# kongqg/marl-sat

Measured on NVIDIA B200. Metric: SATEnv env-steps/s, uf100-430, 1/2/4/8 B200; achieved HBM GB/s vs peak, higher is better.
Workload: dtype u32

## Files before the change

marl_sat_b200/csrc/internal.h:

```cpp
#pragma once
#include <atomic>

#include "common.cuh"

namespace msat {

constexpr int kCtaThreads = 256;
constexpr int kMaxSmemOptin = 227 * 1024;

struct GroupLayout {
    int rec, st, satw, satw_old, x, smx, tt, stage, bar, misc, total;
};
constexpr int kCfStageClauses = 256;
constexpr int kCfStageBytes = 12 * kCfStageClauses + 16;
inline GroupLayout group_layout(const Dims& d, bool obs) {
    GroupLayout L;
    int o = 0;
    const int noobs_rec = d.lits_bytes > d.csr_bytes ? d.lits_bytes : d.csr_bytes;
    L.rec = o;  o += ((obs ? d.rec_copy_bytes : noobs_rec) + 127) & ~127;
    L.st = o;   o += 4 * d.state_words;
    L.stage = o; o += obs ? 0 : kCfStageBytes;
    L.satw = o; o += 4 * d.sw;
    L.satw_old = o; o += 4 * d.sw;
    L.x = o;    o += obs ? 4 * d.xw : 0;
    L.tt = o;   o += ((2 * d.n + 4) & ~3) + 4;
    o = (o + 7) & ~7;
    L.smx = o;  o += obs ? 8 * (d.fw + 2) : 0;
    L.bar = o;  o += 8;
    L.misc = o; o += 16 + 128;
    L.total = (o + 127) & ~127;
    return L;
}

}

struct msat_plan {
    msat::Dims d;
    int group_threads;
    int group_smem_bytes;
    int smem_bytes;
    int group_threads_noobs;
    int smem_bytes_noobs;
    msat::GroupLayout layout_obs, layout_noobs;
    int compile_smem_bytes;
    int requested_group_threads = 0;
    int reward_mode = 0;
    float r_gamma = 0.99f, r_clause = 0.02f, r_sat = 1.0f;
    unsigned long long* reset_counter = nullptr;
    int obs_i8 = 0;
    mutable std::atomic<unsigned long long> prepared_devices{0};
    mutable std::atomic<unsigned long long> prepared_walksat{0};
};

namespace msat {

constexpr int kMaxFusedSteps = 64;

struct EnvArgs {
    GroupLayout L;
    const uint8_t* bank;
    int P;
    const uint32_t* state_in;
    uint32_t* state_out;
    const int32_t* actions;
    const int32_t* prob_idx;
    const uint32_t* keys;
    const uint32_t* rng_in;
    uint32_t* chain_out;
    uint32_t Bg, env_off;
    int auto_reset;
    int32_t* obs;
    int32_t* gnn_assign;
    float* gnn_cf;
    float* reward;
    int reward_cols;
    uint8_t* done;
    int done_cols;
    uint8_t* solved;
    int32_t* num_unsat;
    int32_t* episode_step;
    int B;
    int num_steps;
    long long act_step_stride;
    int emit_every_step;
    int reward_mode;
    float r_gamma, r_clause, r_sat;
    int32_t* newly_sat;
    unsigned long long* reset_count;
    int obs_i8;
    const int32_t* assign_in;
    const int32_t* step_in;
    const uint8_t* done_in;
};

enum EnvMode { MODE_RESET = 0, MODE_STEP = 1, MODE_OBS = 2, MODE_IMPORT = 3 };

extern int g_gae_force_plain;
extern int g_gae_variant;
extern int g_gae_pipe_min_cols;
extern int g_gae_warps_per_sm;

struct ExportArgs {
    const uint8_t* bank;
    int P;
    const uint32_t* state;
    int B;
    int32_t* assign;
    uint8_t* sat;
    int32_t* num_unsat;
    int32_t* step;
    uint8_t* done;
    int32_t* clauses;
// ... 71 lines not shown
```

marl_sat_b200/csrc/satenv.cu:

```cuda
#include <type_traits>

#include "internal.h"

namespace msat {

__global__ void __launch_bounds__(256) compile_bank_kernel(Dims d, const int32_t* __restrict__ clauses,
                                                           uint8_t* __restrict__ bank) {
    extern __shared__ uint32_t csm[];
    uint32_t* clause_agents = csm;
    uint32_t* var_agents = csm + d.m * d.agw;
    const int tid = threadIdx.x, nt = blockDim.x;
    const int32_t* cl = clauses + (size_t)blockIdx.x * d.m * d.k;
    uint8_t* rec = bank + (size_t)blockIdx.x * d.rec_bytes;
    uint16_t* lits = reinterpret_cast<uint16_t*>(rec);
    uint32_t* mflat = reinterpret_cast<uint32_t*>(rec + d.lits_bytes);

    for (int i = tid; i < (d.m + d.n) * d.agw; i += nt) csm[i] = 0u;
    for (int i = tid; i < d.lits_bytes / 2; i += nt) lits[i] = lit_pad(d);
    for (int i = d.lits_bytes / 4 + d.fw + 1 + tid; i < d.rec_bytes / 4; i += nt)
        reinterpret_cast<uint32_t*>(rec)[i] = 0u;
    __syncthreads();

    for (int c = tid; c < d.m; c += nt) {
        uint32_t* ca = clause_agents + c * d.agw;
// ... 22 lines not shown
            const int v = code >> 1;
            for (int w = 0; w < d.agw; ++w) {
                const uint32_t x = clause_agents[c * d.agw + w];
                if (x) atomicOr(&var_agents[v * d.agw + w], x);
            }
        }
    }
    __syncthreads();
    for (int w = tid; w < d.fw + 1; w += nt) {
        uint32_t bits = 0u;
        for (int b = 0; b < 32; ++b) {
            const int j = w * 32 + b;
            if (j >= d.AD) break;
            const int a = j / d.D, p = j - a * d.D;
            uint32_t bit;
            if (p < d.n) {
                bit = var_to_agent(d, p) == a;
            } else if (p < d.n + d.m) {
                bit = (clause_agents[(p - d.n) * d.agw + (a >> 5)] >> (a & 31)) & 1u;
            } else {
                const int v = p - d.n - d.m;
                bit = ((var_agents[v * d.agw + (a >> 5)] >> (a & 31)) & 1u) && var_to_agent(d, v) != a;
            }
            bits |= bit << b;
        }
        mflat[w] = bits;
    }
    if (d.cnt_words) {
        int* cnt = reinterpret_cast<int*>(csm + (d.m + d.n) * d.agw);
        uint16_t* row_off = reinterpret_cast<uint16_t*>(rec + d.csr_off);
        uint16_t* occ = row_off + ((d.n + 1 + 7) & ~7);
        __syncthreads();
        for (int i = tid; i <= d.n; i += nt) cnt[i] = 0;
        __syncthreads();
        for (int i = tid; i < d.m * d.k; i += nt) {
            const uint32_t code = lits[lit_index(d.ms, i / d.k, i % d.k)];
            if (code != lit_pad(d)) atomicAdd(&cnt[code >> 1], 1);
        }
        __syncthreads();
        if (tid == 0) {
            int run = 0;
            for (int v = 0; v < d.n; ++v) {
                const int c = cnt[v];
                cnt[v] = run;
                row_off[v] = (uint16_t)run;
                run += c;
            }
            row_off[d.n] = (uint16_t)run;
        }
        __syncthreads();
        for (int v = tid; v < d.n; v += nt) {
            int o = cnt[v];
            for (int i = 0; i < d.m * d.k; ++i) {
                const int c = i / d.k;
                const uint32_t code = lits[lit_index(d.ms, c, i - c * d.k)];
                if (code != lit_pad(d) && (int)(code >> 1) == v) occ[o++] = (uint16_t)((c << 1) | (code & 1u));
            }
        }
    }
}


template <int GS>
__device__ __forceinline__ void build_truth_table(const Dims& d, const uint32_t* assign, uint8_t* tt, int gt) {
    const int n2 = 2 * d.n;
    for (int w = gt; 4 * w <= n2; w += GS) {
        const int v = 2 * w;
        const uint32_t word = assign[v >> 5] >> (v & 31);
        const uint32_t a0 = word & 1u, a1 = (word >> 1) & 1u;
        uint32_t b = a0 | ((a0 ^ 1u) << 8) | (a1 << 16) | ((a1 ^ 1u) << 24);
        if (v >= d.n) b = 0u;
        else if (v + 1 >= d.n) b &= 0x0000FFFFu;
        reinterpret_cast<uint32_t*>(tt)[w] = b;
    }
}


template <int GS>
__device__ __forceinline__ void publish_unsat(const Dims& d, int* nunsat, int nsat, int gt) {
    if (GS <= 32) *nunsat = d.m - nsat;
    else if ((gt & 31) == 0 && nsat) atomicAdd(nunsat, -nsat);
}

__device__ __forceinline__ void tma_store_1d(void* gmem_dst, const void* smem_src, uint32_t bytes) {
    asm volatile("cp.async.bulk.global.shared::cta.bulk_group [%0], [%1], %2;" ::"l"(gmem_dst), "r"(smem_u32(smem_src)),
                 "r"(bytes)
                 : "memory");
}
__device__ __forceinline__ void tma_store_commit() { asm volatile("cp.async.bulk.commit_group;" ::: "memory"); }
__device__ __forceinline__ void tma_store_wait_read() { asm volatile("cp.async.bulk.wait_group.read 0;" ::: "memory"); }
__device__ __forceinline__ void tma_store_wait() { asm volatile("cp.async.bulk.wait_group 0;" ::: "memory"); }


template <bool K3>
__device__ __forceinline__ uint32_t true_literals(const Dims& d, const uint16_t* lits, const uint8_t* tt, int c) {
    if (K3) {
        const uint32_t l0 = lits[c], l1 = lits[d.ms + c], l2 = lits[2 * d.ms + c];
        return (uint32_t)tt[l0] + tt[l1] + tt[l2];
    }
    uint32_t cnt = 0u;
#pragma unroll 4
    for (int j = 0; j < d.k; ++j) cnt += tt[lits[lit_index(d.ms, c, j)]];
    return cnt;
}

template <bool K3, bool INCR, bool STORE = true>
__device__ __forceinline__ uint32_t clause_count(const Dims& d, const uint16_t* lits, const uint8_t* tt,
                                                 uint32_t* cntw, int c) {
    if (INCR) return (cntw[c >> 3] >> (4 * (c & 7))) & 15u;
    const uint32_t cnt = true_literals<K3>(d, lits, tt, c);
    if (STORE && cntw && cnt) atomicOr(&cntw[c >> 3], cnt << (4 * (c & 7)));
    return cnt;
}

template <int GS, bool K3, bool INCR, bool STORE>
__device__ __forceinline__ void eval_clauses_gnn(const Dims& d, const uint16_t* lits, const uint8_t* tt, uint32_t* cntw,
                                                 uint32_t* satw, int* nunsat, const float2* cf01, uint8_t* stage,
                                                 float* __restrict__ cf_out, int gid, int gt) {
    const int lane = gt & 31;
    int nsat = 0;
    constexpr int kRoundsPerPass = kCfStageClauses / 32;
    const int full = d.m >> 5;
    for (int w0 = 0; w0 < d.sw; w0 += kRoundsPerPass) {
        const int c0 = w0 * 32;
        const int c1 = min(d.m, c0 + kCfStageClauses);
        uint8_t* gdst = reinterpret_cast<uint8_t*>(cf_out + 3 * (size_t)c0);
        const uint32_t phase16 = (uint32_t)(reinterpret_cast<uintptr_t>(gdst) & 15u);
        if (w0 > 0) {
            if (gt == 0) tma_store_wait_read();
            group_sync<GS>(gid);
        }
        const int wend = min(d.sw, w0 + kRoundsPerPass);
        float* o = reinterpret_cast<float*>(stage + phase16) + 3 * (32 * (gt >> 5) + lane);
        int w = w0 + (gt >> 5);
        for (; w < min(wend, full); w += GS / 32, o += 3 * GS) {
            const uint32_t cnt = clause_count<K3, INCR, STORE>(d, lits, tt, cntw, w * 32 + lane);
            const float2 f = cf01[cnt];
            o[0] = f.x;
            o[1] = f.y;
            o[2] = 1.0f;
            const uint32_t word = __ballot_sync(0xffffffffu, cnt != 0u);
            nsat += __popc(word);
            if (lane == 0) satw[w] = word;
        }
        if (w < wend) {
            const int c = w * 32 + lane;
            uint32_t cnt = 0u;
            if (c < d.m) {
                cnt = clause_count<K3, INCR, STORE>(d, lits, tt, cntw, c);
                const float2 f = cf01[cnt];
                o[0] = f.x;
                o[1] = f.y;
                o[2] = 1.0f;
            }
            const uint32_t word = __ballot_sync(0xffffffffu, cnt != 0u);
            nsat += __popc(word);
            if (lane == 0) satw[w] = word;
        }
        fence_proxy_async();
        group_sync<GS>(gid);
        const uint32_t len = 12u * (uint32_t)(c1 - c0);
        uint32_t head = (16u - phase16) & 15u;
        head = head < len ? head : len;
        const uint32_t body = (len - head) & ~15u;
        if (gt == 0 && body) {
            tma_store_1d(gdst + head, stage + phase16 + head, body);
            tma_store_commit();
        }
        if (gt >= 1 && gt < 8) {
            const uint32_t i = gt < 4 ? (uint32_t)(gt - 1) * 4u : head + body + (uint32_t)(gt - 4) * 4u;
            const bool mine = gt < 4 ? i < head : i < len;
            if (mine) *reinterpret_cast<float*>(gdst + i) = *reinterpret_cast<const float*>(stage + phase16 + i);
        }
    }
    publish_unsat<GS>(d, nunsat, nsat, gt);
}

template <int GS, bool CF>
__device__ __forceinline__ void eval_clauses_pairs(const Dims& d, const uint16_t* lits, const uint8_t* tt, int* nunsat,
                                                   const float2* cf01, uint8_t* stage, float* __restrict__ cf_out,
                                                   int gid, int gt) {
    const uint32_t* l32 = reinterpret_cast<const uint32_t*>(lits);
    const int ms2 = d.ms >> 1;
    int nsat = 0;
    auto counts = [&](int pp, uint32_t& ca, uint32_t& cb) {
        const uint32_t w0 = l32[pp], w1 = l32[ms2 + pp], w2 = l32[2 * ms2 + pp];
        ca = (uint32_t)tt[w0 & 0xFFFFu] + tt[w1 & 0xFFFFu] + tt[w2 & 0xFFFFu];
        cb = (uint32_t)tt[w0 >> 16] + tt[w1 >> 16] + tt[w2 >> 16];
        nsat += (ca != 0u) + (cb != 0u);
    };
    if constexpr (!CF) {
        const int npairs = (d.m + 1) >> 1;
        for (int pp = gt; pp < npairs; pp += GS) {
            uint32_t ca, cb;
            counts(pp, ca, cb);
        }
    } else {
        for (int c0 = 0; c0 < d.m; c0 += kCfStageClauses) {
            const int c1 = min(d.m, c0 + kCfStageClauses);
            uint8_t* gdst = reinterpret_cast<uint8_t*>(cf_out + 3 * (size_t)c0);
            const uint32_t phase16 = (uint32_t)(reinterpret_cast<uintptr_t>(gdst) & 15u);
            if (c0 > 0) {
                if (gt == 0) tma_store_wait_read();
                group_sync<GS>(gid);
            }
            const int npass = (c1 - c0 + 1) >> 1;
            const int p0 = c0 >> 1;
            if ((phase16 & 7u) == 0u) {
                for (int q = gt; q < npass; q += GS) {
                    uint32_t ca, cb;
                    counts(p0 + q, ca, cb);
                    const float2 f = cf01[ca], g = cf01[cb];
                    float2* o = reinterpret_cast<float2*>(stage + phase16 + 24 * q);
                    o[0] = f;
                    o[1] = make_float2(1.0f, g.x);
                    o[2] = make_float2(g.y, 1.0f);
                }
            } else {
                for (int q = gt; q < npass; q += GS) {
                    uint32_t ca, cb;
                    counts(p0 + q, ca, cb);
                    const float2 f = cf01[ca], g = cf01[cb];
                    float* o = reinterpret_cast<float*>(stage + phase16 + 24 * q);
                    o[0] = f.x; o[1] = f.y; o[2] = 1.0f;
                    o[3] = g.x; o[4] = g.y; o[5] = 1.0f;
                }
            }
            fence_proxy_async();
            group_sync<GS>(gid);
            const uint32_t len = 12u * (uint32_t)(c1 - c0);
            uint32_t head = (16u - phase16) & 15u;
            head = head < len ? head : len;
            const uint32_t body = (len - head) & ~15u;
            if (gt == 0 && body) {
                tma_store_1d(gdst + head, stage + phase16 + head, body);
                tma_store_commit();
            }
            if (gt >= 1 && gt < 8) {
                const uint32_t i = gt < 4 ? (uint32_t)(gt - 1) * 4u : head + body + (uint32_t)(gt - 4) * 4u;
                const bool mine = gt < 4 ? i < head : i < len;
                if (mine) *reinterpret_cast<float*>(gdst + i) = *reinterpret_cast<const float*>(stage + phase16 + i);
            }
        }
    }
    nsat = __reduce_add_sync(0xffffffffu, nsat);
    if (nunsat) publish_unsat<GS>(d, nunsat, nsat, gt);
}

template <int GS, bool K3, bool INCR, bool STORE>
__device__ __forceinline__ void eval_clauses_impl(const Dims& d, const uint16_t* lits, const uint8_t* tt, uint32_t* cntw,
                                                  uint32_t* satw, int* nunsat, int gt) {
    const int lane = gt & 31;
    int nsat = 0;
    if constexpr (GS < 32) {
        using piece_t = typename std::conditional<GS == 16, uint16_t, uint8_t>::type;
        piece_t* piece = reinterpret_cast<piece_t*>(satw);
        const uint32_t sh = subwarp_shift<GS>();
        const uint32_t mask = subwarp_mask<GS>();
        const int full = d.m / GS;
        int r = 0;
        for (; r < full; ++r) {
            const uint32_t cnt = clause_count<K3, INCR, STORE>(d, lits, tt, cntw, r * GS + gt);
            const uint32_t bits = (__ballot_sync(mask, cnt != 0u) >> sh) & ((1u << GS) - 1u);
            nsat += __popc(bits);
            if (gt == 0) piece[r] = (piece_t)bits;
        }
        if (full * GS < d.m) {
            const int c = r * GS + gt;
            const uint32_t cnt = c < d.m ? clause_count<K3, INCR, STORE>(d, lits, tt, cntw, c) : 0u;
            const uint32_t bits = (__ballot_sync(mask, cnt != 0u) >> sh) & ((1u << GS) - 1u);
            nsat += __popc(bits);
            if (gt == 0) piece[r] = (piece_t)bits;
            ++r;
        }
        if (gt == 0)
            for (; r < (32 / GS) * d.sw; ++r) piece[r] = 0;
    } else {
        for (int w = gt >> 5; w < d.sw; w += GS / 32) {
            const int c = w * 32 + lane;
            const uint32_t cnt = c < d.m ? clause_count<K3, INCR, STORE>(d, lits, tt, cntw, c) : 0u;
            const uint32_t word = __ballot_sync(0xffffffffu, cnt != 0u);
            nsat += __popc(word);
            if (lane == 0) satw[w] = word;
        }
    }
    if (nunsat) publish_unsat<GS>(d, nunsat, nsat, gt);
}
__device__ __forceinline__ uint32_t spread16(uint32_t x) {
    x = (x | (x << 8)) & 0x00FF00FFu;
    x = (x | (x << 4)) & 0x0F0F0F0Fu;
    x = (x | (x << 2)) & 0x33333333u;
    return (x | (x << 1)) & 0x55555555u;
}
__device__ __forceinline__ void eval_clauses_pairs16(const Dims& d, const uint16_t* lits, const uint8_t* tt,
                                                     uint32_t* satw, int* nunsat, int gt) {
    const uint32_t* l32 = reinterpret_cast<const uint32_t*>(lits);
    const int ms2 = d.ms >> 1;
    const uint32_t sh = subwarp_shift<16>();
    const uint32_t mask = subwarp_mask<16>();
    int nsat = 0;
    for (int w = 0; w < d.sw; ++w) {
        const int pp = 16 * w + gt;
        uint32_t ca = 0u, cb = 0u;
        if (pp < ms2) {
            const uint32_t w0 = l32[pp], w1 = l32[ms2 + pp], w2 = l32[2 * ms2 + pp];
            ca = (uint32_t)tt[w0 & 0xFFFFu] + tt[w1 & 0xFFFFu] + tt[w2 & 0xFFFFu];
            cb = (uint32_t)tt[w0 >> 16] + tt[w1 >> 16] + tt[w2 >> 16];
        }
        const uint32_t ev = (__ballot_sync(mask, ca != 0u) >> sh) & 0xFFFFu;
        const uint32_t od = (__ballot_sync(mask, cb != 0u) >> sh) & 0xFFFFu;
        const uint32_t word = spread16(ev) | (spread16(od) << 1);
        nsat += __popc(word);
        if (gt == 0) satw[w] = word;
    }
    if (nunsat) publish_unsat<16>(d, nunsat, nsat, gt);
}

template <int GS, bool K3, bool INCR>
__device__ __forceinline__ void eval_clauses(const Dims& d, const uint16_t* lits, const uint8_t* tt, uint32_t* cntw,
                                             uint32_t* satw, int* nunsat, int gt) {
    if constexpr (GS == 16 && K3 && !INCR) {
        if (!cntw && d.sw >= 4) {
            eval_clauses_pairs16(d, lits, tt, satw, nunsat, gt);
            return;
// ... 144 lines not shown
        smx[w] = make_uint2(mw, xw);
    }
    group_sync<GS>(gid);

    if constexpr (I8) {
        int8_t* out8 = reinterpret_cast<int8_t*>(obs) + (g_start - s);
        const int lo = s, hi = s + d.AD;
        const int q_lo = (lo + 15) >> 4, q_hi = hi >> 4;
        {
            int q = q_lo + gt;
            const int sh = (q & 1) * 16;
            const uint2* sp = smx + (q >> 1);
            uint4* op = reinterpret_cast<uint4*>(out8) + q;
#pragma unroll 2
            for (; q < q_hi; q += GS, sp += GS / 2, op += GS) {
                const uint2 mx = *sp;
                const uint32_t m16 = mx.x >> sh, x16 = mx.y >> sh;
                __stcs(op, make_uint4(expand_nibble_i8(m16 & 0xFu, x16 & 0xFu),
                                      expand_nibble_i8((m16 >> 4) & 0xFu, (x16 >> 4) & 0xFu),
                                      expand_nibble_i8((m16 >> 8) & 0xFu, (x16 >> 8) & 0xFu),
                                      expand_nibble_i8((m16 >> 12) & 0xFu, (x16 >> 12) & 0xFu)));
            }
        }
        const int head_end = min(16 * q_lo, hi);
        const int tail_start = max(16 * q_hi, head_end);
        auto put = [&](int i) {
            const uint2 mx = smx[i >> 5];
            out8[i] = ((mx.x >> (i & 31)) & 1u) ? (int8_t)((mx.y >> (i & 31)) & 1u) : (int8_t)-1;
        };
        for (int i = lo + gt; i < head_end; i += GS) put(i);
        for (int i = tail_start + gt; i < hi; i += GS) put(i);
        return;
    }
    int32_t* out = obs + (g_start - s);
    const int lo_valid = s, hi_valid = s + d.AD;
    const int q_lo = (lo_valid + 3) >> 2;
    const int q_hi = hi_valid >> 2;
    {
        int q = q_lo + gt;
        const int sh = (q & 7) * 4;
        const uint2* sp = smx + (q >> 3);
        int4* op = reinterpret_cast<int4*>(out) + q;
#pragma unroll 4
        for (; q < q_hi; q += GS, sp += GS / 8, op += GS) {
            const uint2 mx = *sp;
            __stcs(op, expand_nibble((mx.x >> sh) & 0xFu, (mx.y >> sh) & 0xFu));
        }
    }
    if (gt < 8) {
        const int q = (gt < 4) ? q_lo - 1 : q_hi;
        const int i = 4 * q + (gt & 3);
        const bool partial = (gt < 4) ? (4 * q_lo != lo_valid) : (4 * q_hi != hi_valid);
        if (partial && q >= 0 && i >= lo_valid && i < hi_valid) {
            const uint2 mx = smx[i >> 5];
            out[i] = ((mx.x >> (i & 31)) & 1u) ? (int)((mx.y >> (i & 31)) & 1u) : -1;
        }
    }
}

template <int GS, typename F>
__device__ __forceinline__ void store_words_vec4(uint32_t* __restrict__ dst, int count, int gt, F f) {
    int head = (int)(((16u - (uint32_t)(reinterpret_cast<uintptr_t>(dst) & 15u)) & 15u) >> 2);
    head = head < count ? head : count;
    const int n4 = (count - head) >> 2;
    uint4* d4 = reinterpret_cast<uint4*>(dst + head);
    for (int q = gt; q < n4; q += GS) {
        const int i = head + 4 * q;
        __stcs(d4 + q, make_uint4(f(i), f(i + 1), f(i + 2), f(i + 3)));
    }
    if (gt < head) dst[gt] = f(gt);
    const int i = head + 4 * n4 + gt;
    if (gt < 3 && i < count) dst[i] = f(i);
}

template <int GS>
__device__ __forceinline__ void emit_gnn_assignment(const Dims& d, long long row, const uint32_t* assign,
                                                    int32_t* __restrict__ gnn_assign, int gt) {
    store_words_vec4<GS>(reinterpret_cast<uint32_t*>(gnn_assign) + row * d.n, d.n, gt,
                         [&](int v) { return (assign[v >> 5] >> (v & 31)) & 1u; });
}

template <int GS, bool INCR, bool OBS>
__device__ __forceinline__ void run_eval(const Dims& d, const uint16_t* lits, const uint8_t* tt, uint32_t* cntw,
                                         uint32_t* satw, int* nunsat, const float2* cf01, uint8_t* stage, float* cf_row,
                                         bool pairs, int gid, int gt) {
    if constexpr (!OBS && !INCR && GS >= 32) {
        if (pairs) {
            if (cf_row) eval_clauses_pairs<GS, true>(d, lits, tt, nunsat, cf01, stage, cf_row, gid, gt);
            else eval_clauses_pairs<GS, false>(d, lits, tt, nunsat, cf01, stage, cf_row, gid, gt);
            return;
        }
    }
    if (GS >= 32 && cf_row) {
        if constexpr (GS >= 32) {
            const bool store = !INCR && cntw != nullptr;
            if (d.k == 3) {
                if (store) eval_clauses_gnn<GS, true, INCR, true>(d, lits, tt, cntw, satw, nunsat, cf01, stage, cf_row, gid, gt);
                else eval_clauses_gnn<GS, true, INCR, false>(d, lits, tt, cntw, satw, nunsat, cf01, stage, cf_row, gid, gt);
            } else {
                if (store) eval_clauses_gnn<GS, false, INCR, true>(d, lits, tt, cntw, satw, nunsat, cf01, stage, cf_row, gid, gt);
                else eval_clauses_gnn<GS, false, INCR, false>(d, lits, tt, cntw, satw, nunsat, cf01, stage, cf_row, gid, gt);
            }
        }
    } else {
        if (d.k == 3) eval_clauses<GS, true, INCR>(d, lits, tt, cntw, satw, nunsat, gt);
        else eval_clauses<GS, false, INCR>(d, lits, tt, cntw, satw, nunsat, gt);
    }
}

__device__ __forceinline__ void rng_advance(uint32_t& r0, uint32_t& r1) {
    uint32_t a[2], b[2];
    split2(r0, r1, a, b);
    split2(a[0], a[1], a, b);
    uint32_t x0 = 0u, x1 = 3u, y0 = 1u, y1 = 4u;
    threefry2x32(a[0], a[1], x0, x1);
    threefry2x32(a[0], a[1], y0, y1);
    r0 = x0;
    r1 = y0;
}

template <int GS, int MODE, bool OBS, bool MULTI, bool INCR>
__global__ void __launch_bounds__(kCtaThreads, (MULTI || !OBS) ? 4 : 8) env_kernel(const Dims d, const EnvArgs a) {
    extern __shared__ __align__(128) uint8_t smem_raw[];
    constexpr int NG = kCtaThreads / GS;
    constexpr bool FRESH = MODE == MODE_RESET || MODE == MODE_IMPORT;
    const int gid = threadIdx.x / GS, gt = threadIdx.x % GS;
    const int e = blockIdx.x * NG + gid;
    const GroupLayout& L = a.L;
    const int K = MULTI ? a.num_steps : 1;

    uint32_t* s_chain = reinterpret_cast<uint32_t*>(smem_raw + (size_t)NG * L.total);
    if (MULTI && a.rng_in) {
        if (threadIdx.x == 0) {
            uint32_t r0 = a.rng_in[0], r1 = a.rng_in[1];
            for (int j = 0; j < K; ++j) {
                s_chain[10 * j] = r0;
                s_chain[10 * j + 1] = r1;
                rng_advance(r0, r1);
            }
        }
        __syncthreads();
        if ((int)threadIdx.x < K) {
            uint32_t c[10];
            rng_chain_compute(s_chain[10 * threadIdx.x], s_chain[10 * threadIdx.x + 1], c);
            for (int i = 0; i < 10; ++i) s_chain[10 * threadIdx.x + i] = c[i];
        }
        __syncthreads();
        if (blockIdx.x == 0 && threadIdx.x < 10) a.chain_out[threadIdx.x] = s_chain[10 * (K - 1) + threadIdx.x];
    }
    if (e >= a.B) return;

    uint8_t* base = smem_raw + (size_t)gid * L.total;
    uint8_t* rec = base + L.rec;
    uint32_t* st = reinterpret_cast<uint32_t*>(base + L.st);
    uint32_t* satw = reinterpret_cast<uint32_t*>(base + L.satw);
    uint32_t* satw_old = reinterpret_cast<uint32_t*>(base + L.satw_old);
    uint32_t* X = reinterpret_cast<uint32_t*>(base + L.x);
    uint2* smx = reinterpret_cast<uint2*>(base + L.smx);
    uint8_t* tt = base + L.tt;
    uint8_t* stage = base + L.stage;
    uint64_t* bar = reinterpret_cast<uint64_t*>(base + L.bar);
    int* misc = reinterpret_cast<int*>(base + L.misc);
    const uint16_t* lits = reinterpret_cast<const uint16_t*>(rec);
    const uint32_t* mflat = reinterpret_cast<const uint32_t*>(rec + d.lits_bytes);
    uint32_t* st_tail = st + d.aw;
    const uint32_t tma_bytes = OBS ? (uint32_t)d.rec_copy_bytes : (uint32_t)d.lits_bytes;
    uint32_t* cntw = d.cnt_words ? st + d.aw + 4 : nullptr;
    uint32_t* cnt_store = (MODE != MODE_OBS) ? cntw : nullptr;
    const bool want_cf = !OBS && a.gnn_cf != nullptr;
    const bool pairs = !OBS && d.k == 3 && cnt_store == nullptr && cntw == nullptr && a.reward_mode == 0;
    float2* cf01 = reinterpret_cast<float2*>(misc + 4);

    const uint4* sin = FRESH ? nullptr : reinterpret_cast<const uint4*>(a.state_in + (size_t)e * d.state_words);
    const int sw4 = d.state_words >> 2;
    uint4 s0 = make_uint4(0u, 0u, 0u, 0u);
    if (!FRESH && gt < sw4) s0 = sin[gt];
    if constexpr (GS < 32) {
        if (gt < sw4) reinterpret_cast<uint4*>(st)[gt] = s0;
    }
    int act_pre = 0;
    const bool act_pre_ok = GS >= 32 && MODE == MODE_STEP && !INCR && d.action_mode == 0 && gt < d.A;
    if (act_pre_ok) act_pre = a.actions[(size_t)e * d.A + gt];
    if (gt == 0) {
        misc[0] = d.m;
        mbar_init(bar, 1);
    }
    if (want_cf && gt < 16) cf01[gt] = make_float2(gt > 0 ? 1.0f : 0.0f, __fdiv_rn((float)gt, 3.0f));
    if constexpr (GS >= 32) {
        if (gt < sw4) reinterpret_cast<uint4*>(st)[gt] = s0;
    }
    if (!FRESH) {
#pragma unroll 1
        for (int i = gt + GS; i < sw4; i += GS) reinterpret_cast<uint4*>(st)[i] = sin[i];
    } else {
#pragma unroll 1
        for (int i = gt + GS; i < sw4; i += GS) reinterpret_cast<uint4*>(st)[i] = make_uint4(0u, 0u, 0u, 0u);
    }
    group_sync<GS>(gid);

    int step_cur = (MODE == MODE_RESET) ? 0
                 : (MODE == MODE_IMPORT) ? (a.step_in ? a.step_in[e] : 0) : (int)st_tail[ST_STEP];
    int nunsat_prev = FRESH ? 0 : (int)st_tail[ST_NUNSAT];
    uint32_t flags = (MODE == MODE_RESET) ? 0u
                   : (MODE == MODE_IMPORT) ? ((a.done_in && a.done_in[e]) ? 1u : 0u) : st_tail[ST_FLAGS];
    int pidx;
    if (FRESH) pidx = a.prob_idx[e];
    else pidx = (int)st_tail[ST_PIDX];
    pidx = clamp_problem(pidx, a.P);
    int loaded_pidx = -1;
    bool loaded_csr = false;
    uint32_t phase = 0u;
    int nunsat = nunsat_prev;

    for (int j = 0; j < K; ++j) {
        const bool last = j == K - 1;
        const bool emit = last || a.emit_every_step;
        const long long row = (a.emit_every_step ? (long long)j * a.B : 0LL) + e;
        const long long orow = (long long)j * a.B + e;

        if (!INCR && loaded_pidx != pidx && gt == 0) {
            if (j > 0) fence_proxy_async();
            mbar_expect_tx(bar, tma_bytes);
            tma_load_1d(rec, a.bank + (size_t)pidx * d.rec_bytes, tma_bytes, bar);
        }
        const bool need_csr = INCR && !(loaded_csr && loaded_pidx == pidx);
        if (need_csr && gt == 0) {
            if (j > 0) fence_proxy_async();
            mbar_expect_tx(bar, (uint32_t)d.csr_bytes);
            tma_load_1d(rec, a.bank + (size_t)pidx * d.rec_bytes + d.csr_off, (uint32_t)d.csr_bytes, bar);
        }
        if (MODE == MODE_STEP && a.reward_mode) {
            if (INCR) {
                run_eval<GS, true, OBS>(d, lits, tt, cntw, satw_old, nullptr, cf01, stage, nullptr, false, gid, gt);
            } else {
                if (loaded_pidx != pidx) {
                    mbar_wait(bar, phase);
                    phase ^= 1u;
                    loaded_pidx = pidx;
                }
                build_truth_table<GS>(d, st, tt, gt);
                group_sync<GS>(gid);
                run_eval<GS, false, OBS>(d, lits, tt, nullptr, satw_old, nullptr, cf01, stage, nullptr, false, gid, gt);
            }
            group_sync<GS>(gid);
        }

        if (MODE == MODE_RESET) {
            threefry_assign<GS>(d, a.keys[2 * (size_t)e], a.keys[2 * (size_t)e + 1], st, gt);
        } else if (MODE == MODE_IMPORT) {
            load_assign<GS>(d, a.assign_in + (size_t)e * d.n, st, gt);
        } else if (MODE == MODE_STEP) {
            if (INCR) {
                if (need_csr) {
                    mbar_wait(bar, phase);
                    phase ^= 1u;
                    loaded_pidx = pidx;
                    loaded_csr = true;
                }
                for_each_flip<GS>(d, a.actions + (long long)j * a.act_step_stride, e, gt, false, 0,
                                  [&](int v) { flip_and_update_counts(d, rec, v, st, cntw); });
            } else {
                for_each_flip<GS>(d, a.actions + (long long)j * a.act_step_stride, e, gt, act_pre_ok && j == 0, act_pre,
                                  [&](int v) { atomicXor(&st[v >> 5], 1u << (v & 31)); });
            }
        }
        if (!INCR && cnt_store)
            for (int i = gt; i < d.cnt_words; i += GS) cnt_store[i] = 0u;
        group_sync<GS>(gid);
        if (!INCR) {
            build_truth_table<GS>(d, st, tt, gt);
            if (loaded_pidx != pidx) {
                mbar_wait(bar, phase);
                phase ^= 1u;
                loaded_pidx = pidx;
            }
            group_sync<GS>(gid);
        }

        float* cf_row = (want_cf && emit) ? a.gnn_cf + row * d.m * 3 : nullptr;
        run_eval<GS, INCR, OBS>(d, lits, tt, INCR ? cntw : cnt_store, satw, &misc[0], cf01, stage, cf_row, pairs, gid, gt);
        group_sync<GS>(gid);
        nunsat = misc[0];

        if (MODE == MODE_STEP) {
            if (!MULTI && a.rng_in && blockIdx.x == 0 && threadIdx.x == 0) {
                uint32_t c[10];
                rng_chain_compute(a.rng_in[0], a.rng_in[1], c);
                for (int i = 0; i < 10; ++i) a.chain_out[i] = c[i];
            }
            const bool solved = nunsat == 0;
            const bool done = solved || (step_cur + 1 >= d.max_steps);
            int newly = 0;
            float r = solved ? 1.0f : 0.0f;
            if (a.reward_mode) {
                for (int w = 0; w < d.sw; ++w) newly += __popc(satw[w] & ~satw_old[w]);
                const float r_pbrs = __fsub_rn(__fmul_rn(a.r_gamma, (float)(-nunsat)), (float)(-nunsat_prev));
                const float r_cl = __fmul_rn((float)newly, a.r_clause);
                r = __fadd_rn(__fadd_rn(r_pbrs, r_cl), solved ? a.r_sat : 0.0f);
            }
            if (a.reward) {
                float* rp = a.reward + orow * a.reward_cols;
#pragma unroll 1
                for (int i = gt; i < a.reward_cols; i += GS) rp[i] = r;
            }
            if (a.done) {
                uint8_t* dp = a.done + orow * a.done_cols;
#pragma unroll 1
                for (int i = gt; i < a.done_cols; i += GS) dp[i] = done ? 1 : 0;
            }
            if (gt == 0) {
                if (a.solved) a.solved[orow] = solved ? 1 : 0;
                if (a.num_unsat) a.num_unsat[orow] = nunsat;
                if (a.episode_step) a.episode_step[orow] = step_cur + 1;
                if (a.newly_sat) a.newly_sat[orow] = newly;
            }
            if (done && a.auto_reset) {
                group_sync<GS>(gid);
                uint32_t rk0, rk1;
                if (a.rng_in) {
                    if (gt < 4) {
                        const int base_lane = GS < 32 ? (int)(threadIdx.x & 31u & (32u - GS)) : 0;
                        uint32_t c6 = 0u, c7 = 0u, c8 = 0u, c9 = 0u, r0 = 0u, r1 = 0u, np, k0, k1;
                        if (MULTI) {
                            c6 = s_chain[10 * j + 6]; c7 = s_chain[10 * j + 7];
                            c8 = s_chain[10 * j + 8]; c9 = s_chain[10 * j + 9];
                        } else {
                            r0 = a.rng_in[0]; r1 = a.rng_in[1];
                        }
                        env_reset_inputs_4lanes(0xFu << base_lane, gt, base_lane, MULTI, r0, r1, c6, c7, c8, c9, a.Bg,
                                                a.env_off + (uint32_t)e, (uint32_t)a.P, np, k0, k1);
                        if (gt == 0) {
                            misc[1] = (int)np;
                            misc[2] = (int)k0;
                            misc[3] = (int)k1;
                        }
                    }
                    group_sync<GS>(gid);
                    pidx = misc[1];
                    rk0 = (uint32_t)misc[2];
                    rk1 = (uint32_t)misc[3];
                } else {
                    pidx = a.prob_idx[e];
                    rk0 = a.keys[2 * (size_t)e];
                    rk1 = a.keys[2 * (size_t)e + 1];
                }
                pidx = clamp_problem(pidx, a.P);
                const bool need_lits = pidx != loaded_pidx || (INCR && loaded_csr);
                if (gt == 0) {
                    misc[0] = d.m;
                    if (a.reset_count) atomicAdd(a.reset_count, 1ULL);
                    if (need_lits) {
                        fence_proxy_async();
                        mbar_expect_tx(bar, tma_bytes);
                        tma_load_1d(rec, a.bank + (size_t)pidx * d.rec_bytes, tma_bytes, bar);
                    }
                }
                for (int i = gt; i < d.aw; i += GS) st[i] = 0u;
                if (cnt_store)
                    for (int i = gt; i < d.cnt_words; i += GS) cnt_store[i] = 0u;
                group_sync<GS>(gid);
                threefry_assign<GS>(d, rk0, rk1, st, gt);
                group_sync<GS>(gid);
                build_truth_table<GS>(d, st, tt, gt);
                if (need_lits) {
                    mbar_wait(bar, phase);
                    phase ^= 1u;
                    loaded_pidx = pidx;
                    loaded_csr = false;
                }
                group_sync<GS>(gid);
                if (cf_row) {
                    if (gt == 0) tma_store_wait();
                    group_sync<GS>(gid);
                }
                run_eval<GS, false, OBS>(d, lits, tt, cnt_store, satw, &misc[0], cf01, stage, cf_row, pairs, gid, gt);
                group_sync<GS>(gid);
                nunsat = misc[0];
                step_cur = 0;
                flags = 0u;
            } else {
                step_cur += 1;
                flags = done ? 1u : 0u;
            }
            nunsat_prev = nunsat;
        }
        if (emit) {
            if (!OBS && a.gnn_assign) emit_gnn_assignment<GS>(d, row, st, a.gnn_assign, gt);
            if (OBS && a.obs) {
                if (a.obs_i8) emit_obs<GS, true>(d, row, st, satw, X, smx, mflat, a.obs, gid, gt);
                else emit_obs<GS, false>(d, row, st, satw, X, smx, mflat, a.obs, gid, gt);
            }
        }
        if (!last) {
            if (cf_row && gt == 0) tma_store_wait_read();
            group_sync<GS>(gid);
            if (gt == 0) misc[0] = d.m;
        }
    }

    if (want_cf && gt == 0) tma_store_wait_read();
    if (MODE != MODE_OBS) {
        group_sync<GS>(gid);
        if (gt == 0) {
            st_tail[ST_STEP] = (uint32_t)step_cur;
            st_tail[ST_PIDX] = (uint32_t)pidx;
            st_tail[ST_NUNSAT] = (uint32_t)nunsat;
            st_tail[ST_FLAGS] = flags;
        }
        group_sync<GS>(gid);
        uint4* sout = reinterpret_cast<uint4*>(a.state_out + (size_t)e * d.state_words);
#pragma unroll 1
        for (int i = gt; i < (d.state_words >> 2); i += GS) sout[i] = reinterpret_cast<const uint4*>(st)[i];
    }
}

template <int GS, bool OBS>
static cudaError_t launch_env_gs(const msat_plan* plan, EnvMode mode, const EnvArgs& a, cudaStream_t s, int smem_bytes) {
    const int groups = kCtaThreads / GS;
    const int grid = (a.B + groups - 1) / groups;
    if (grid == 0) return cudaSuccess;
    constexpr int kFns = OBS ? 5 : 7;
    const void* fns[7] = {(const void*)env_kernel<GS, MODE_RESET, OBS, false, false>,
                          (const void*)env_kernel<GS, MODE_STEP, OBS, false, false>,
                          (const void*)env_kernel<GS, MODE_OBS, OBS, false, false>,
                          (const void*)env_kernel<GS, MODE_IMPORT, OBS, false, false>,
                          (const void*)env_kernel<GS, MODE_STEP, OBS, true, false>,
                          OBS ? nullptr : (const void*)env_kernel<GS, MODE_STEP, false, false, true>,
                          OBS ? nullptr : (const void*)env_kernel<GS, MODE_STEP, false, true, true>};
    const bool multi = mode == MODE_STEP && a.num_steps > 1;
    const bool incr = !OBS && mode == MODE_STEP && plan->d.cnt_words > 0;
    if (multi) smem_bytes += 40 * a.num_steps;
    if (smem_bytes > 48 * 1024) {
        int dev = 0;
        cudaError_t err = cudaGetDevice(&dev);
        if (err != cudaSuccess) return err;
        const unsigned long long bit = 1ULL << ((OBS ? 0 : 32) + (dev & 31));
        if (!(plan->prepared_devices.load(std::memory_order_acquire) & bit)) {
            for (int i = 0; i < kFns; ++i) {
                err = cudaFuncSetAttribute(fns[i], cudaFuncAttributeMaxDynamicSharedMemorySize, kMaxSmemOptin);
                if (err != cudaSuccess) return err;
            }
            plan->prepared_devices.fetch_or(bit, std::memory_order_release);
        }
    }
    const void* fn = fns[incr ? 5 + (int)multi : (multi ? 4 : (int)mode)];
    Dims d = plan->d;
    EnvArgs args = a;
    void* params[] = {&d, &args};
    return cudaLaunchKernel(fn, dim3(grid), dim3(kCtaThreads), params, (size_t)smem_bytes, s);
}

cudaError_t launch_env(const msat_plan* plan, EnvMode mode, const EnvArgs& a0, cudaStream_t s) {
    EnvArgs a = a0;
    if (a.num_steps < 1) a.num_steps = 1;
    const bool noobs = a.obs == nullptr;
    a.L = noobs ? plan->layout_noobs : plan->layout_obs;
    a.obs_i8 = plan->obs_i8;
    const int gs = noobs ? plan->group_threads_noobs : plan->group_threads;
    const int smem = noobs ? plan->smem_bytes_noobs : plan->smem_bytes;
    if (noobs) {
        switch (gs) {
            case 32: return launch_env_gs<32, false>(plan, mode, a, s, smem);
            case 64: return launch_env_gs<64, false>(plan, mode, a, s, smem);
            case 128: return launch_env_gs<128, false>(plan, mode, a, s, smem);
            default: return launch_env_gs<256, false>(plan, mode, a, s, smem);
        }
    }
    switch (gs) {
        case 16: return launch_env_gs<16, true>(plan, mode, a, s, smem);
        case 32: return launch_env_gs<32, true>(plan, mode, a, s, smem);
        case 64: return launch_env_gs<64, true>(plan, mode, a, s, smem);
        case 128: return launch_env_gs<128, true>(plan, mode, a, s, smem);
        default: return launch_env_gs<256, true>(plan, mode, a, s, smem);
    }
}

cudaError_t launch_compile_bank(const msat_plan* plan, const int32_t* clauses, int P, uint8_t* bank, cudaStream_t s) {
    if (P == 0) return cudaSuccess;
    if (plan->compile_smem_bytes > 48 * 1024) {
        cudaError_t err = cudaFuncSetAttribute((const void*)compile_bank_kernel,
                                               cudaFuncAttributeMaxDynamicSharedMemorySize, plan->compile_smem_bytes);
        if (err != cudaSuccess) return err;
    }
// ... 62 lines not shown
```

Baseline: 121.7 million.

## Replace TMA-staged clause-feature stores with direct streaming stores and shrink smem

Clause features for the GNN outputs used to be staged in a shared-memory buffer and written out with bulk-async (TMA) stores, with group syncs and wait-group fences between chunks. They are now written straight to global memory with streaming (__stcs) stores, using float2 stores when the output is 8-byte aligned. This drops the staging buffer and its synchronisation, which shrinks the per-group shared-memory footprint, and the non-obs launch bound is raised from 4 to 6 blocks per SM. Other changes: the cf lookup table now comes from a constant array, and the RNG chain computation moves to kernel entry on the non-obs step path. The cost is scattered 4/8-byte stores in place of coalesced bulk copies, and possible register pressure from the higher occupancy target.

```diff
diff --git a/marl_sat_b200/csrc/internal.h b/marl_sat_b200/csrc/internal.h
--- a/marl_sat_b200/csrc/internal.h
+++ b/marl_sat_b200/csrc/internal.h
@@ -9,17 +9,15 @@
 constexpr int kMaxSmemOptin = 227 * 1024;
 
 struct GroupLayout {
-    int rec, st, satw, satw_old, x, smx, tt, stage, bar, misc, total;
+    int rec, st, satw, satw_old, x, smx, tt, cf, bar, misc, total;
 };
-constexpr int kCfStageClauses = 256;
-constexpr int kCfStageBytes = 12 * kCfStageClauses + 16;
 inline GroupLayout group_layout(const Dims& d, bool obs) {
     GroupLayout L;
     int o = 0;
     const int noobs_rec = d.lits_bytes > d.csr_bytes ? d.lits_bytes : d.csr_bytes;
     L.rec = o;  o += ((obs ? d.rec_copy_bytes : noobs_rec) + 127) & ~127;
     L.st = o;   o += 4 * d.state_words;
-    L.stage = o; o += obs ? 0 : kCfStageBytes;
+    L.cf = o;   o += obs ? 0 : 128;
     L.satw = o; o += 4 * d.sw;
     L.satw_old = o; o += 4 * d.sw;
     L.x = o;    o += obs ? 4 * d.xw : 0;
@@ -27,7 +25,7 @@
     o = (o + 7) & ~7;
     L.smx = o;  o += obs ? 8 * (d.fw + 2) : 0;
     L.bar = o;  o += 8;
-    L.misc = o; o += 16 + 128;
+    L.misc = o; o += 16;
     L.total = (o + 127) & ~127;
     return L;
 }
diff --git a/marl_sat_b200/csrc/satenv.cu b/marl_sat_b200/csrc/satenv.cu
--- a/marl_sat_b200/csrc/satenv.cu
+++ b/marl_sat_b200/csrc/satenv.cu
@@ -128,16 +128,6 @@
     else if ((gt & 31) == 0 && nsat) atomicAdd(nunsat, -nsat);
 }
 
-__device__ __forceinline__ void tma_store_1d(void* gmem_dst, const void* smem_src, uint32_t bytes) {
-    asm volatile("cp.async.bulk.global.shared::cta.bulk_group [%0], [%1], %2;" ::"l"(gmem_dst), "r"(smem_u32(smem_src)),
-                 "r"(bytes)
-                 : "memory");
-}
-__device__ __forceinline__ void tma_store_commit() { asm volatile("cp.async.bulk.commit_group;" ::: "memory"); }
-__device__ __forceinline__ void tma_store_wait_read() { asm volatile("cp.async.bulk.wait_group.read 0;" ::: "memory"); }
-__device__ __forceinline__ void tma_store_wait() { asm volatile("cp.async.bulk.wait_group 0;" ::: "memory"); }
-
-
 template <bool K3>
 __device__ __forceinline__ uint32_t true_literals(const Dims& d, const uint16_t* lits, const uint8_t* tt, int c) {
     if (K3) {
@@ -149,6 +139,11 @@
     for (int j = 0; j < d.k; ++j) cnt += tt[lits[lit_index(d.ms, c, j)]];
     return cnt;
 }
+
+__constant__ float2 kCf01[16] = {{0.f, 0.f / 3.f},  {1.f, 1.f / 3.f},  {1.f, 2.f / 3.f},  {1.f, 3.f / 3.f},
+                                 {1.f, 4.f / 3.f},  {1.f, 5.f / 3.f},  {1.f, 6.f / 3.f},  {1.f, 7.f / 3.f},
+                                 {1.f, 8.f / 3.f},  {1.f, 9.f / 3.f},  {1.f, 10.f / 3.f}, {1.f, 11.f / 3.f},
+                                 {1.f, 12.f / 3.f}, {1.f, 13.f / 3.f}, {1.f, 14.f / 3.f}, {1.f, 15.f / 3.f}};
 
 template <bool K3, bool INCR, bool STORE = true>
 __device__ __forceinline__ uint32_t clause_count(const Dims& d, const uint16_t* lits, const uint8_t* tt,
@@ -161,131 +156,61 @@
 
 template <int GS, bool K3, bool INCR, bool STORE>
 __device__ __forceinline__ void eval_clauses_gnn(const Dims& d, const uint16_t* lits, const uint8_t* tt, uint32_t* cntw,
-                                                 uint32_t* satw, int* nunsat, const float2* cf01, uint8_t* stage,
-                                                 float* __restrict__ cf_out, int gid, int gt) {
+                                                 uint32_t* satw, int* nunsat, const float2* cf01,
+                                                 float* __restrict__ cf_out, int gt) {
     const int lane = gt & 31;
     int nsat = 0;
-    constexpr int kRoundsPerPass = kCfStageClauses / 32;
-    const int full = d.m >> 5;
-    for (int w0 = 0; w0 < d.sw; w0 += kRoundsPerPass) {
-        const int c0 = w0 * 32;
-        const int c1 = min(d.m, c0 + kCfStageClauses);
-        uint8_t* gdst = reinterpret_cast<uint8_t*>(cf_out + 3 * (size_t)c0);
-        const uint32_t phase16 = (uint32_t)(reinterpret_cast<uintptr_t>(gdst) & 15u);
-        if (w0 > 0) {
-            if (gt == 0) tma_store_wait_read();
-            group_sync<GS>(gid);
-        }
-        const int wend = min(d.sw, w0 + kRoundsPerPass);
-        float* o = reinterpret_cast<float*>(stage + phase16) + 3 * (32 * (gt >> 5) + lane);
-        int w = w0 + (gt >> 5);
-        for (; w < min(wend, full); w += GS / 32, o += 3 * GS) {
-            const uint32_t cnt = clause_count<K3, INCR, STORE>(d, lits, tt, cntw, w * 32 + lane);
+    for (int w = gt >> 5; w < d.sw; w += GS / 32) {
+        const int c = w * 32 + lane;
+        uint32_t cnt = 0u;
+        if (c < d.m) {
+            cnt = clause_count<K3, INCR, STORE>(d, lits, tt, cntw, c);
             const float2 f = cf01[cnt];
-            o[0] = f.x;
-            o[1] = f.y;
-            o[2] = 1.0f;
-            const uint32_t word = __ballot_sync(0xffffffffu, cnt != 0u);
-            nsat += __popc(word);
-            if (lane == 0) satw[w] = word;
-        }
-        if (w < wend) {
-            const int c = w * 32 + lane;
-            uint32_t cnt = 0u;
-            if (c < d.m) {
-                cnt = clause_count<K3, INCR, STORE>(d, lits, tt, cntw, c);
-                const float2 f = cf01[cnt];
-                o[0] = f.x;
-                o[1] = f.y;
-                o[2] = 1.0f;
-            }
-            const uint32_t word = __ballot_sync(0xffffffffu, cnt != 0u);
-            nsat += __popc(word);
-            if (lane == 0) satw[w] = word;
-        }
-        fence_proxy_async();
-        group_sync<GS>(gid);
-        const uint32_t len = 12u * (uint32_t)(c1 - c0);
-        uint32_t head = (16u - phase16) & 15u;
-        head = head < len ? head : len;
-        const uint32_t body = (len - head) & ~15u;
-        if (gt == 0 && body) {
-            tma_store_1d(gdst + head, stage + phase16 + head, body);
-            tma_store_commit();
-        }
-        if (gt >= 1 && gt < 8) {
-            const uint32_t i = gt < 4 ? (uint32_t)(gt - 1) * 4u : head + body + (uint32_t)(gt - 4) * 4u;
-            const bool mine = gt < 4 ? i < head : i < len;
-            if (mine) *reinterpret_cast<float*>(gdst + i) = *reinterpret_cast<const float*>(stage + phase16 + i);
-        }
+            __stcs(cf_out + 3 * c, f.x);
+            __stcs(cf_out + 3 * c + 1, f.y);
+            __stcs(cf_out + 3 * c + 2, 1.0f);
+        }
+        const uint32_t word = __ballot_sync(0xffffffffu, cnt != 0u);
+        nsat += __popc(word);
+        if (lane == 0) satw[w] = word;
     }
     publish_unsat<GS>(d, nunsat, nsat, gt);
 }
 
 template <int GS, bool CF>
 __device__ __forceinline__ void eval_clauses_pairs(const Dims& d, const uint16_t* lits, const uint8_t* tt, int* nunsat,
-                                                   const float2* cf01, uint8_t* stage, float* __restrict__ cf_out,
-                                                   int gid, int gt) {
+                                                   const float2* cf01, float* __restrict__ cf_out, int gt) {
     const uint32_t* l32 = reinterpret_cast<const uint32_t*>(lits);
     const int ms2 = d.ms >> 1;
+    const int npairs = (d.m + 1) >> 1;
+    const bool al8 = (reinterpret_cast<uintptr_t>(cf_out) & 7u) == 0u;
     int nsat = 0;
-    auto counts = [&](int pp, uint32_t& ca, uint32_t& cb) {
+    for (int pp = gt; pp < npairs; pp += GS) {
         const uint32_t w0 = l32[pp], w1 = l32[ms2 + pp], w2 = l32[2 * ms2 + pp];
-        ca = (uint32_t)tt[w0 & 0xFFFFu] + tt[w1 & 0xFFFFu] + tt[w2 & 0xFFFFu];
-        cb = (uint32_t)tt[w0 >> 16] + tt[w1 >> 16] + tt[w2 >> 16];
+        const uint32_t ca = (uint32_t)tt[w0 & 0xFFFFu] + tt[w1 & 0xFFFFu] + tt[w2 & 0xFFFFu];
+        const uint32_t cb = (uint32_t)tt[w0 >> 16] + tt[w1 >> 16] + tt[w2 >> 16];
         nsat += (ca != 0u) + (cb != 0u);
-    };
-    if constexpr (!CF) {
-        const int npairs = (d.m + 1) >> 1;
-        for (int pp = gt; pp < npairs; pp += GS) {
-            uint32_t ca, cb;
-            counts(pp, ca, cb);
-        }
-    } else {
-        for (int c0 = 0; c0 < d.m; c0 += kCfStageClauses) {
-            const int c1 = min(d.m, c0 + kCfStageClauses);
-            uint8_t* gdst = reinterpret_cast<uint8_t*>(cf_out + 3 * (size_t)c0);
-            const uint32_t phase16 = (uint32_t)(reinterpret_cast<uintptr_t>(gdst) & 15u);
-            if (c0 > 0) {
-                if (gt == 0) tma_store_wait_read();
-                group_sync<GS>(gid);
-            }
-            const int npass = (c1 - c0 + 1) >> 1;
-            const int p0 = c0 >> 1;
-            if ((phase16 & 7u) == 0u) {
-                for (int q = gt; q < npass; q += GS) {
-                    uint32_t ca, cb;
-                    counts(p0 + q, ca, cb);
-                    const float2 f = cf01[ca], g = cf01[cb];
-                    float2* o = reinterpret_cast<float2*>(stage + phase16 + 24 * q);
-                    o[0] = f;
-                    o[1] = make_float2(1.0f, g.x);
-                    o[2] = make_float2(g.y, 1.0f);
+        if constexpr (CF) {
+            const float2 f = cf01[ca], g = cf01[cb];
+            float* o = cf_out + 6 * pp;
+            const bool two = 2 * pp + 1 < d.m;
+            if (al8) {
+                __stcs(reinterpret_cast<float2*>(o), f);
+                if (two) {
+                    __stcs(reinterpret_cast<float2*>(o) + 1, make_float2(1.0f, g.x));
+                    __stcs(reinterpret_cast<float2*>(o) + 2, make_float2(g.y, 1.0f));
+                } else {
+                    __stcs(o + 2, 1.0f);
                 }
             } else {
-                for (int q = gt; q < npass; q += GS) {
-                    uint32_t ca, cb;
-                    counts(p0 + q, ca, cb);
-                    const float2 f = cf01[ca], g = cf01[cb];
-                    float* o = reinterpret_cast<float*>(stage + phase16 + 24 * q);
-                    o[0] = f.x; o[1] = f.y; o[2] = 1.0f;
-                    o[3] = g.x; o[4] = g.y; o[5] = 1.0f;
+                __stcs(o, f.x);
+                __stcs(o + 1, f.y);
+                __stcs(o + 2, 1.0f);
+                if (two) {
+                    __stcs(o + 3, g.x);
+                    __stcs(o + 4, g.y);
+                    __stcs(o + 5, 1.0f);
                 }
-            }
-            fence_proxy_async();
-            group_sync<GS>(gid);
-            const uint32_t len = 12u * (uint32_t)(c1 - c0);
-            uint32_t head = (16u - phase16) & 15u;
-            head = head < len ? head : len;
-            const uint32_t body = (len - head) & ~15u;
-            if (gt == 0 && body) {
-                tma_store_1d(gdst + head, stage + phase16 + head, body);
-                tma_store_commit();
-            }
-            if (gt >= 1 && gt < 8) {
-                const uint32_t i = gt < 4 ? (uint32_t)(gt - 1) * 4u : head + body + (uint32_t)(gt - 4) * 4u;
-                const bool mine = gt < 4 ? i < head : i < len;
-                if (mine) *reinterpret_cast<float*>(gdst + i) = *reinterpret_cast<const float*>(stage + phase16 + i);
             }
         }
     }
@@ -596,12 +521,12 @@
 
 template <int GS, bool INCR, bool OBS>
 __device__ __forceinline__ void run_eval(const Dims& d, const uint16_t* lits, const uint8_t* tt, uint32_t* cntw,
-                                         uint32_t* satw, int* nunsat, const float2* cf01, uint8_t* stage, float* cf_row,
-                                         bool pairs, int gid, int gt) {
+                                         uint32_t* satw, int* nunsat, const float2* cf01, float* cf_row, bool pairs,
+                                         int gt) {
     if constexpr (!OBS && !INCR && GS >= 32) {
         if (pairs) {
-            if (cf_row) eval_clauses_pairs<GS, true>(d, lits, tt, nunsat, cf01, stage, cf_row, gid, gt);
-            else eval_clauses_pairs<GS, false>(d, lits, tt, nunsat, cf01, stage, cf_row, gid, gt);
+            if (cf_row) eval_clauses_pairs<GS, true>(d, lits, tt, nunsat, cf01, cf_row, gt);
+            else eval_clauses_pairs<GS, false>(d, lits, tt, nunsat, cf01, cf_row, gt);
             return;
         }
     }
@@ -609,11 +534,11 @@
         if constexpr (GS >= 32) {
             const bool store = !INCR && cntw != nullptr;
             if (d.k == 3) {
-                if (store) eval_clauses_gnn<GS, true, INCR, true>(d, lits, tt, cntw, satw, nunsat, cf01, stage, cf_row, gid, gt);
-                else eval_clauses_gnn<GS, true, INCR, false>(d, lits, tt, cntw, satw, nunsat, cf01, stage, cf_row, gid, gt);
+                if (store) eval_clauses_gnn<GS, true, INCR, true>(d, lits, tt, cntw, satw, nunsat, cf01, cf_row, gt);
+                else eval_clauses_gnn<GS, true, INCR, false>(d, lits, tt, cntw, satw, nunsat, cf01, cf_row, gt);
             } else {
-                if (store) eval_clauses_gnn<GS, false, INCR, true>(d, lits, tt, cntw, satw, nunsat, cf01, stage, cf_row, gid, gt);
-                else eval_clauses_gnn<GS, false, INCR, false>(d, lits, tt, cntw, satw, nunsat, cf01, stage, cf_row, gid, gt);
+                if (store) eval_clauses_gnn<GS, false, INCR, true>(d, lits, tt, cntw, satw, nunsat, cf01, cf_row, gt);
+                else eval_clauses_gnn<GS, false, INCR, false>(d, lits, tt, cntw, satw, nunsat, cf01, cf_row, gt);
             }
         }
     } else {
@@ -634,7 +559,7 @@
 }
 
 template <int GS, int MODE, bool OBS, bool MULTI, bool INCR>
-__global__ void __launch_bounds__(kCtaThreads, (MULTI || !OBS) ? 4 : 8) env_kernel(const Dims d, const EnvArgs a) {
+__global__ void __launch_bounds__(kCtaThreads, MULTI ? 4 : (OBS ? 8 : 6)) env_kernel(const Dims d, const EnvArgs a) {
     extern __shared__ __align__(128) uint8_t smem_raw[];
     constexpr int NG = kCtaThreads / GS;
     constexpr bool FRESH = MODE == MODE_RESET || MODE == MODE_IMPORT;
@@ -642,6 +567,12 @@
     const int e = blockIdx.x * NG + gid;
     const GroupLayout& L = a.L;
     const int K = MULTI ? a.num_steps : 1;
+
+    if (!OBS && MODE == MODE_STEP && !MULTI && a.rng_in && blockIdx.x == 0 && threadIdx.x == 0) {
+        uint32_t c[10];
+        rng_chain_compute(a.rng_in[0], a.rng_in[1], c);
+        for (int i = 0; i < 10; ++i) a.chain_out[i] = c[i];
+    }
 
     uint32_t* s_chain = reinterpret_cast<uint32_t*>(smem_raw + (size_t)NG * L.total);
     if (MULTI && a.rng_in) {
@@ -672,7 +603,6 @@
     uint32_t* X = reinterpret_cast<uint32_t*>(base + L.x);
     uint2* smx = reinterpret_cast<uint2*>(base + L.smx);
     uint8_t* tt = base + L.tt;
-    uint8_t* stage = base + L.stage;
     uint64_t* bar = reinterpret_cast<uint64_t*>(base + L.bar);
     int* misc = reinterpret_cast<int*>(base + L.misc);
     const uint16_t* lits = reinterpret_cast<const uint16_t*>(rec);
@@ -683,7 +613,7 @@
     uint32_t* cnt_store = (MODE != MODE_OBS) ? cntw : nullptr;
     const bool want_cf = !OBS && a.gnn_cf != nullptr;
     const bool pairs = !OBS && d.k == 3 && cnt_store == nullptr && cntw == nullptr && a.reward_mode == 0;
-    float2* cf01 = reinterpret_cast<float2*>(misc + 4);
+    float2* cf01 = reinterpret_cast<float2*>(base + L.cf);
 
     const uint4* sin = FRESH ? nullptr : reinterpret_cast<const uint4*>(a.state_in + (size_t)e * d.state_words);
     const int sw4 = d.state_words >> 2;
@@ -699,7 +629,7 @@
         misc[0] = d.m;
         mbar_init(bar, 1);
     }
-    if (want_cf && gt < 16) cf01[gt] = make_float2(gt > 0 ? 1.0f : 0.0f, __fdiv_rn((float)gt, 3.0f));
+    if (want_cf && gt < 16) cf01[gt] = kCf01[gt];
     if constexpr (GS >= 32) {
         if (gt < sw4) reinterpret_cast<uint4*>(st)[gt] = s0;
     }
@@ -745,7 +675,7 @@
         }
         if (MODE == MODE_STEP && a.reward_mode) {
             if (INCR) {
-                run_eval<GS, true, OBS>(d, lits, tt, cntw, satw_old, nullptr, cf01, stage, nullptr, false, gid, gt);
+                run_eval<GS, true, OBS>(d, lits, tt, cntw, satw_old, nullptr, cf01, nullptr, false, gt);
             } else {
                 if (loaded_pidx != pidx) {
                     mbar_wait(bar, phase);
@@ -754,7 +684,7 @@
                 }
                 build_truth_table<GS>(d, st, tt, gt);
                 group_sync<GS>(gid);
-                run_eval<GS, false, OBS>(d, lits, tt, nullptr, satw_old, nullptr, cf01, stage, nullptr, false, gid, gt);
+                run_eval<GS, false, OBS>(d, lits, tt, nullptr, satw_old, nullptr, cf01, nullptr, false, gt);
             }
             group_sync<GS>(gid);
         }
@@ -792,12 +722,12 @@
         }
 
         float* cf_row = (want_cf && emit) ? a.gnn_cf + row * d.m * 3 : nullptr;
-        run_eval<GS, INCR, OBS>(d, lits, tt, INCR ? cntw : cnt_store, satw, &misc[0], cf01, stage, cf_row, pairs, gid, gt);
+        run_eval<GS, INCR, OBS>(d, lits, tt, INCR ? cntw : cnt_store, satw, &misc[0], cf01, cf_row, pairs, gt);
         group_sync<GS>(gid);
         nunsat = misc[0];
 
         if (MODE == MODE_STEP) {
-            if (!MULTI && a.rng_in && blockIdx.x == 0 && threadIdx.x == 0) {
+            if (OBS && !MULTI && a.rng_in && blockIdx.x == 0 && threadIdx.x == 0) {
                 uint32_t c[10];
                 rng_chain_compute(a.rng_in[0], a.rng_in[1], c);
                 for (int i = 0; i < 10; ++i) a.chain_out[i] = c[i];
@@ -883,11 +813,7 @@
                     loaded_csr = false;
                 }
                 group_sync<GS>(gid);
-                if (cf_row) {
-                    if (gt == 0) tma_store_wait();
-                    group_sync<GS>(gid);
-                }
-                run_eval<GS, false, OBS>(d, lits, tt, cnt_store, satw, &misc[0], cf01, stage, cf_row, pairs, gid, gt);
+                run_eval<GS, false, OBS>(d, lits, tt, cnt_store, satw, &misc[0], cf01, cf_row, pairs, gt);
                 group_sync<GS>(gid);
                 nunsat = misc[0];
                 step_cur = 0;
@@ -906,13 +832,11 @@
             }
         }
         if (!last) {
-            if (cf_row && gt == 0) tma_store_wait_read();
             group_sync<GS>(gid);
             if (gt == 0) misc[0] = d.m;
         }
     }
 
-    if (want_cf && gt == 0) tma_store_wait_read();
     if (MODE != MODE_OBS) {
         group_sync<GS>(gid);
         if (gt == 0) {
diff --git a/profiles/gnn_step_ab.py b/profiles/gnn_step_ab.py
--- /dev/null
+++ b/profiles/gnn_step_ab.py
@@ -0,0 +1,141 @@
+from __future__ import annotations
+
+import argparse
+import hashlib
+import json
+import os
+import statistics
+import subprocess
+import sys
+
+sys.dont_write_bytecode = True
+ROOT = os.path.dirname(os.path.dirname(os.path.abspath(__file__)))
+N, M_, K, ENVS, MAX_STEPS, SEED, ACTION_CYCLE = 100, 430, 3, 65536, 512, 42, 64
+
+
+def digest(tree: str, steps: int) -> dict:
+    sys.path.insert(0, os.path.abspath(tree))
+    import torch
+
+    import marl_sat_b200 as M
+    from marl_sat_b200 import synth
+    assert os.path.dirname(os.path.abspath(M.__file__)) == os.path.join(os.path.abspath(tree), "marl_sat_b200")
+    dev = "cuda:0"
+    env = M.SATEnv(N, M_, MAX_STEPS, verbose=False, device=dev)
+    problems = synth.uniform_ksat_torch(ENVS, N, M_, K, seed=20261018 + 2, device=dev)
+    bank = env.make_bank(problems, validate=False)
+    gen = torch.Generator(device=dev).manual_seed(SEED)
+    A, V = env.num_agents, env.max_vars_per_agent
+    actions = torch.randint(0, V + 1, (ACTION_CYCLE, ENVS, A), generator=gen, device=dev, dtype=torch.int32)
+    vec = M.VecSATEnv(env, bank, ENVS, M.prng_key(SEED + 2), emit_obs=False, compact_outputs=True, gnn_outputs=True)
+    vec.reset()
+    g = torch.arange(ENVS, device=dev, dtype=torch.int64)
+    vec.set_episode_steps((g % MAX_STEPS).to(torch.int32))
+    rows = []
+    for t in range(steps):
+        out = vec.step(actions[t % ACTION_CYCLE])
+        torch.cuda.synchronize()
+        rows.append({
+            "assignment": hashlib.sha256(out["gnn_assignment"].cpu().numpy().tobytes()).hexdigest(),
+            "clause_features": hashlib.sha256(out["gnn_clause_features"].cpu().numpy().tobytes()).hexdigest(),
+            "episodes_ended": int(out["done"].reshape(ENVS, -1)[:, -1].sum()),
+        })
+    return {"tree": os.path.abspath(tree), "steps": rows}
+
+
+def card() -> dict:
+    import torch
+    info = {"name": torch.cuda.get_device_name(), "power_limit": "unknown", "max_sm_clock": "unknown"}
+    try:
+        out = subprocess.run(["nvidia-smi", "--query-gpu=power.limit,clocks.max.sm", "--format=csv,noheader", "-i", "0"],
+                             capture_output=True, text=True, timeout=30)
+        info["power_limit"], info["max_sm_clock"] = [s.strip() for s in out.stdout.strip().split(",")]
+    except Exception:
+        pass
+    return info
+
+
+def legs(line: dict) -> dict:
+    g = line.get("gnn_input_mode", {})
+    cv = g.get("clause_update_variants", {})
+    out = {"gnn_input_mode": g.get("ms_per_step")}
+    for label in ("gnn_input", "state_only"):
+        for variant in ("full", "incremental"):
+            out[f"{label}.{variant}"] = cv.get(label, {}).get(f"{variant}_ms_per_step")
+    out["value"] = line.get("value")
+    out["obs_int8_mode"] = line.get("obs_int8_mode", {}).get("ms_per_step")
+    e2e = line.get("e2e")
+    out["e2e"] = e2e.get("value") if isinstance(e2e, dict) else e2e
+    return out
+
+
+def bench(tree: str) -> dict:
+    res = subprocess.run([sys.executable, "bench.py", "--no-cpu-baseline"], cwd=tree, capture_output=True, text=True)
+    if res.returncode != 0:
+        raise SystemExit(f"bench.py failed in {tree}:\n{res.stdout[-3000:]}\n{res.stderr[-3000:]}")
+    line = json.loads([s for s in res.stdout.splitlines() if s.startswith("{")][-1])
+    return legs(line)
+
+
+def summary(xs):
+    xs = [x for x in xs if x is not None]
+    return {"median": statistics.median(xs), "min": min(xs), "max": max(xs), "runs": xs} if xs else None
+
+
+def compare(args) -> dict:
+    trees = {"parent": os.path.abspath(args.parent), "this": ROOT}
+    digests = {}
+    for name, tree in trees.items():
+        res = subprocess.run([sys.executable, os.path.abspath(__file__), "digest", "--tree", tree, "--steps",
+                              str(args.steps)], capture_output=True, text=True)
+        if res.returncode != 0:
+            raise SystemExit(f"digest of {tree} failed:\n{res.stdout[-3000:]}\n{res.stderr[-3000:]}")
+        digests[name] = json.loads(res.stdout.strip().splitlines()[-1])["steps"]
+    identical = digests["parent"] == digests["this"]
+    runs = {"parent": [], "this": []}
+    for p in range(args.pairs):
+        for name in (("parent", "this") if p % 2 == 0 else ("this", "parent")):
+            runs[name].append(bench(trees[name]))
+            print(name, runs[name][-1], flush=True)
+    keys = list(runs["parent"][0])
+    result = {
+        "card": card(),
+        "gnn_outputs_identical": identical,
+        "episodes_ended_per_step": [r["episodes_ended"] for r in digests["this"]],
+        "digests": digests,
+        "bench_pairs": args.pairs,
+        "units": "ms per step; value and e2e in env-steps/s",
+        "parent": {k: summary([r[k] for r in runs["parent"]]) for k in keys},
+        "this": {k: summary([r[k] for r in runs["this"]]) for k in keys},
+    }
+    if not identical:
+        print("GNN outputs differ between the builds", file=sys.stderr)
+    return result
+
+
+def main():
+    ap = argparse.ArgumentParser()
+    ap.add_argument("what", choices=["digest", "compare"])
+    ap.add_argument("--tree", default=ROOT)
+    ap.add_argument("--parent", default=None)
+    ap.add_argument("--steps", type=int, default=12)
+    ap.add_argument("--pairs", type=int, default=3)
+    ap.add_argument("--out", default=None)
+    args = ap.parse_args()
+    if args.what == "digest":
+        print(json.dumps(digest(args.tree, args.steps)))
+        return
+    if not args.parent:
+        raise SystemExit("compare needs --parent")
+    result = compare(args)
+    text = json.dumps(result, indent=1)
+    if args.out:
+        with open(args.out, "w") as f:
+            f.write(text + "\n")
+    print(text)
+    if not result["gnn_outputs_identical"]:
+        raise SystemExit(1)
+
+
+if __name__ == "__main__":
+    main()
```

Result: no change. 121.7 million, median of 6 (-0.0%).
